# jedisct1/zig-lz4

Measured on AMD Instinct MI355X. Metric: GiB/s uncompressed, block compress+decompress, higher is better.
Workload: dtype u8

## Files before the change

### zig-lz4_amd/csrc/zlz4_compress_dict.hip

```cpp
#include "zlz4_device.hpp"

namespace zlz4 {

namespace {

__device__ __forceinline__ uint32_t dc_hash4(uint32_t seq) { return (seq * kHashMul) >> 20; }

__device__ __forceinline__ uint32_t dc_skip_sum(uint32_t x) {
    const uint32_t q = x >> 6, r = x & 63u;
    return 32u * q * (q - 1u) + q * r;
}

__device__ __forceinline__ int64_t dc_last_literals(uint8_t *dst, uint32_t dst_len, uint32_t op, const uint8_t *lit_src,
                                                    uint32_t lit, uint32_t lane) {
    if (lit == 0) return (int64_t)op;
    const uint32_t nle = ext_len_bytes(lit);
    if ((uint64_t)op + 1u + nle + lit > dst_len) return kErrOutputTooSmall;
    if (lane == 0) dst[op] = (uint8_t)((lit >= 15u ? 15u : lit) << 4);
    if (lit >= 15u) write_ext_len(dst + op + 1u, lit, lane);
    copy_bytes(dst + op + 1u + nle, lit_src, lit, lane);
    return (int64_t)(op + 1u + nle + lit);
}

struct VBuf {
// ... 275 lines not shown
                    if (x >= 64u) {
                        if (nseq == 0u) continue_generic = true;
                        break;
                    }
                    uint64_t pm = 0;
                    if (xp >> 7) {
                        const uint64_t grp_x = (uint64_t)rdlane((uint32_t)grp, x) | ((uint64_t)rdlane((uint32_t)(grp >> 32), x) << 32);
                        pm = grp_x & wrmask & ~covered_now() & ((1ull << x) - 1ull);
                    }
                    const uint32_t j = x;
                    const uint32_t m_pos = A + j;
                    uint32_t m_cand, mlen;
                    if (pm) {
                        const uint32_t pr = 63u - (uint32_t)__builtin_clzll(pm);
                        if (rdlane(fwd.x, pr) != rdlane(fwd.x, x)) { f = x + 1u; continue; }
                        m_cand = A + pr;
                        const uint64_t xa = ((uint64_t)(rdlane(fwd.z, j) ^ rdlane(fwd.z, pr)) << 32) | (rdlane(fwd.y, j) ^ rdlane(fwd.y, pr));
                        const uint32_t xb = rdlane(fwd.w, j) ^ rdlane(fwd.w, pr);
                        if (xa) mlen = (uint32_t)__builtin_ctzll(xa) >> 3;
                        else if (xb) mlen = 8u + ((uint32_t)__builtin_ctz(xb) >> 3);
                        else mlen = dc_extend_match(V, m_pos, m_cand, 12u, match_limit, lane);
                    } else {
                        const uint32_t q = rdlane(Q, x);
                        if (!(q & 1u)) { f = x + 1u; continue; }
                        mlen = q >> 1;
                        if (mlen < 44u && !tight) {
                            mm_run |= 1ull << j;
                            nseq++;
                            a = j + kMinMatch + mlen;
                            if (a >= 64u) break;
                            f = a + 1u;
                            continue;
                        }
                        m_cand = rdlane(old, x);
                        if (mlen >= 44u) mlen = dc_extend_match(V, m_pos, m_cand, 44u, match_limit, lane);
                    }
                    const uint32_t lit = j - a;
                    const uint32_t offset = m_pos - m_cand;
                    const uint32_t e = j + kMinMatch + mlen;
                    if (!tight && mlen < 270u) {
                        v_end = wrlane(e, j, v_end);
                        mlo_e = wrlane(mlen, j, mlo_e);
                        off_e = wrlane(offset, j, off_e);
                        mm_run |= 1ull << j;
                        nseq++;
                        a = e;
                        if (e >= 64u) break;
                        f = e + 1u;
                        continue;
                    }
                    if (mm_run) flush_run();
                    const uint32_t nle = ext_len_bytes(lit), nme = ext_len_bytes(mlen);
                    const uint64_t seq_end = (uint64_t)op + 1u + nle + lit + 2u + nme;
                    if (seq_end > dst_len) { failed = true; break; }
                    if (lane == 0)
                        dst[op] = (uint8_t)(((lit >= 15u ? 15u : lit) << 4) | (mlen >= 15u ? 15u : mlen));
                    if (lit >= 15u) write_ext_len(dst + op + 1u, lit, lane);
                    uint8_t *o = dst + op + 1u + nle;
                    if (lane >= a && lane < j) o[lane - a] = (uint8_t)fwd.x;
                    o += lit;
                    if (lane < 2u) o[lane] = (uint8_t)(offset >> (8u * lane));
                    if (mlen >= 15u) write_ext_len(o + 2u, mlen, lane);
                    op = (uint32_t)seq_end;
                    {
                        const uint64_t upto_e = e >= 64u ? ~0ull : (1ull << e) - 1ull;
                        covered_x |= upto_e & ~((2ull << j) - 1ull);
                    }
                    nseq++;
                    a = e;
                    if (e >= 64u) break;
                    f = e + 1u;
                }
                const bool next_win = !continue_generic && !failed && a != 0u && (uint64_t)A + a + 192u < L;
                if (next_win) {
                    pf_anchor = A + a;
                    fwd_pf = ld128(V.srcv + pf_anchor + lane);
                }
                if (mm_run && !failed) flush_run();
                anchor = A + a;
                const uint32_t f_end = continue_generic ? 64u : (a >= 64u ? 64u : a + 1u);
                const uint64_t ins = wrmask & ~covered_now() & (f_end >= 64u ? ~0ull : (1ull << f_end) - 1ull);
                if (failed) break;
                if (wr && !(ins & lane_bit)) table[h] = (T)old;
                __builtin_amdgcn_fence(__ATOMIC_RELEASE, "wavefront");
                if ((ins & lane_bit) && (grp & ins & ~lanes_below & ~lane_bit) == 0) table[h] = (T)mine;
                __builtin_amdgcn_fence(__ATOMIC_RELEASE, "wavefront");
                moved = anchor != A;
                to_generic = continue_generic;
                if (next_win) {
                    has_ins = true;
                    F0 = anchor + 1u;
                    if (++guard > src_size) { failed = true; break; }
                    continue;
                }
                break;
              }
                if (failed) break;
                if (!to_generic && moved) {
                    if (anchor < L) { has_ins = true; F0 = anchor + 1u; }
                    else { has_ins = false; F0 = L; }
                    continue;
                }
                if (to_generic) ub = 63;
            }

            bool found = false;
            uint32_t m_pos = 0, m_cand = 0, m_local = 0;
            bool m_local_done = false;
            for (;;) {
                const int32_t u = ub + (int32_t)lane;
                uint32_t pos, step_next;
                if (u <= 0) {
                    pos = (u < 0) ? F0 - 1u : F0;
                    step_next = accel;
                } else if (u == 1) {
                    pos = F0 + accel;
                    step_next = accel >> 6;
                } else {
                    const uint32_t x = cbase + (uint32_t)u - 1u;
                    pos = F0 + accel + dc_skip_sum(x) - s_cbase;
                    step_next = x >> 6;
                }
                const bool is_probe = u >= 0;
                const bool bail = is_probe && ((uint64_t)pos + step_next > L);
                const uint64_t bail_mask = ballot(bail);
                const uint32_t nb = bail_mask ? first_lane(bail_mask) : 64u;
                const bool active = lane < nb;

                const bool have16 = active && (pos + 16u <= V.end);
                u32x4 fwd = {0, 0, 0, 0};
                if (have16) fwd = ld128(V.srcv + pos);
                else if (active) fwd.x = ld32(V.srcv + pos);
                const uint32_t h = dc_hash4(fwd.x);
                const uint32_t mine = (uint32_t)(T)pos;

                uint32_t old = 0, rb = 0;
                if (active) {
                    old = table[h];
                    table[h] = (T)mine;
                }
                __builtin_amdgcn_fence(__ATOMIC_RELEASE, "wavefront");
                if (active) rb = table[h];
                uint64_t losers = ballot(active && rb != mine);
                uint64_t grp = lane_bit;
                int32_t pred = -1;
                while (losers) {
                    const uint32_t l = first_lane(losers);
                    const uint32_t hh = rdlane(h, l);
                    const uint64_t same = ballot(active && h == hh);
                    if (active && h == hh) {
                        grp = same;
                        const uint64_t below = same & lanes_below;
                        pred = below ? 63 - (int32_t)__clzll((long long)below) : -1;
                    }
                    losers &= ~same;
                }
                const uint32_t pred_pos = shfl(pos, (uint32_t)(pred < 0 ? 0 : pred));
                const uint32_t cand = pred >= 0 ? pred_pos : old;

                bool valid = is_probe && active && cand > 0 && cand < pos && (cand + kMaxDist >= pos);
                u32x4 cnd = {0, 0, 0, 0};
                bool cnd16 = false;
                if (valid) {
                    cnd16 = have16 && V.whole(cand, 16u);
                    if (cnd16) cnd = ld128(V.at(cand)); else cnd.x = V.rd32(cand);
                    valid = cnd.x == fwd.x;
                }
                const uint64_t valid_mask = ballot(valid);

                if (valid_mask) {
                    const uint32_t wl = first_lane(valid_mask);
                    if (active && lane > wl) table[h] = (T)old;
                    __builtin_amdgcn_fence(__ATOMIC_RELEASE, "wavefront");
                    const uint64_t upto = (2ull << wl) - 1ull;
                    if (active && lane <= wl && ((grp & upto & ~lanes_below & ~lane_bit) == 0)) table[h] = (T)mine;
                    __builtin_amdgcn_fence(__ATOMIC_RELEASE, "wavefront");
                    uint32_t loc = 0;
                    bool loc_done = false;
                    if (lane == wl && cnd16) {
                        const uint32_t lim = match_limit - (pos + kMinMatch);
                        u32x4 a = fwd, b = cnd;
                        a.x = 0; b.x = 0;
                        loc = first_diff16(a, b) - 4u;
                        if (loc >= lim) { loc = lim; loc_done = true; }
                        else if (loc < 12u) loc_done = true;
                    }
                    m_pos = rdlane(pos, wl);
                    m_cand = rdlane(cand, wl);
                    m_local = rdlane(loc, wl);
                    m_local_done = rdlane((uint32_t)loc_done, wl) != 0;
                    found = true;
                    break;
                }
                if (bail_mask) break;
                if (active && ((grp & ~lanes_below & ~lane_bit) == 0) && grp != lane_bit) table[h] = (T)mine;
                __builtin_amdgcn_fence(__ATOMIC_RELEASE, "wavefront");
                ub += 64;
            }
            if (!found) break;

            const uint32_t mlen = m_local_done ? m_local : dc_extend_match(V, m_pos, m_cand, m_local, match_limit, lane);

            const uint32_t lit = m_pos - anchor;
            const uint32_t nle = ext_len_bytes(lit), nme = ext_len_bytes(mlen);
            const uint64_t seq_end = (uint64_t)op + 1u + nle + lit + 2u + nme;
            if (seq_end > dst_len) { failed = true; break; }
            if (lane == 0)
                dst[op] = (uint8_t)(((lit >= 15u ? 15u : lit) << 4) | (mlen >= 15u ? 15u : mlen));
            if (lit >= 15u) write_ext_len(dst + op + 1u, lit, lane);
            uint8_t *o = dst + op + 1u + nle;
            copy_bytes(o, V.srcv + anchor, lit, lane);
            o += lit;
            const uint32_t offset = m_pos - m_cand;
            if (lane < 2u) o[lane] = (uint8_t)(offset >> (8u * lane));
            if (mlen >= 15u) write_ext_len(o + 2u, mlen, lane);
            op = (uint32_t)seq_end;

            const uint32_t end = m_pos + kMinMatch + mlen;
            anchor = end;
            if (end < L) { has_ins = true; F0 = end + 1u; }
            else { has_ins = false; F0 = L; }
        }
        res = failed ? kErrOutputTooSmall
                     : dc_last_literals(dst, dst_len, op, V.srcv + anchor, V.end - anchor, lane);
    }
    if (lane == 0) d_result[blk] = res;
}

}

extern "C" int zlz4_launch_compress_fast_using_dict(hipStream_t stream, const uint8_t *d_in, const uint64_t *d_in_off,
                                                    const uint32_t *d_in_len, uint8_t *d_out, const uint64_t *d_out_off,
                                                    const uint32_t *d_out_cap, const uint8_t *d_dict,
                                                    const uint64_t *d_dict_off, const uint32_t *d_dict_len,
                                                    const uint32_t *d_table, const uint32_t *d_table_idx, int64_t *d_result,
                                                    uint32_t nblocks, uint32_t max_in_len, uint32_t max_dict_len,
                                                    uint32_t acceleration) {
    if (nblocks == 0) return 0;
    const uint32_t dmax = max_dict_len < 65536u ? max_dict_len : 65536u;
#define ZLZ4_LAUNCH_DICT(T)                                                                                              \
    hipLaunchKernelGGL((zlz4::k_compress_fast_dict<T>), dim3(nblocks), dim3(64), 4096 * sizeof(T), stream, d_in, d_in_off, \
                       d_in_len, d_out, d_out_off, d_out_cap, d_dict, d_dict_off, d_dict_len, d_table, d_table_idx,        \
                       d_result, nblocks, max_in_len, dmax, acceleration)
    if ((uint64_t)dmax + max_in_len <= 65536u + 11u) ZLZ4_LAUNCH_DICT(uint16_t);
    else ZLZ4_LAUNCH_DICT(uint32_t);
#undef ZLZ4_LAUNCH_DICT
    return hipGetLastError() == hipSuccess ? 0 : -7;
}
```

### zig-lz4_amd/csrc/zlz4_compress_fast.hip

```cpp
#include <cstdlib>

#include "zlz4_device.hpp"

#ifdef ZLZ4_STAMPS
__device__ unsigned long long g_zlz4_stamps[24];
#define STAMP_DECL unsigned long long st_acc[24] = {0,0,0,0,0,0,0,0,0,0,0,0,0,0,0,0,0,0,0,0,0,0,0,0}; unsigned long long st_last = __builtin_amdgcn_s_memtime();
#define STAMP(i) do { unsigned long long st_now; __builtin_amdgcn_sched_barrier(0); \
                      asm volatile("s_memtime %0\n\ts_waitcnt lgkmcnt(0)" : "=s"(st_now) :: "memory"); \
                      __builtin_amdgcn_sched_barrier(0); st_acc[i] += st_now - st_last; st_last = st_now; } while (0)
#define STAMP_COUNT(i) do { st_acc[i] += 1; } while (0)
#define STAMP_FLUSH do { if (lane == 0) for (int st_k = 0; st_k < 24; st_k++) atomicAdd(&g_zlz4_stamps[st_k], st_acc[st_k]); } while (0)
#else
#define STAMP_DECL
#define STAMP(i)
#define STAMP_COUNT(i)
#define STAMP_FLUSH
#endif

namespace zlz4 {

__device__ __forceinline__ uint32_t hash4(uint32_t seq) { return (seq * kHashMul) >> 20; }

__device__ __forceinline__ uint32_t skip_sum(uint32_t x) {
    const uint32_t q = x >> 6, r = x & 63u;
// ... 84 lines not shown
                }
                for (int q = 0; q < 4; q++) table[4u * k + q] = (T)e[q];
            }
            __builtin_amdgcn_fence(__ATOMIC_RELEASE, "wavefront");
        } else {
        {
            u32x4 z = {0, 0, 0, 0};
            u32x4 *t4 = reinterpret_cast<u32x4 *>(lds_raw) + wave_in_wg * (4096u * sizeof(T) / 16u);
            const uint32_t n16 = 4096u * sizeof(T) / 16u;
            for (uint32_t k = lane; k < n16; k += 64u) t4[k] = z;
        }
        }
        const uint32_t accel = acceleration < 1u ? 1u : (acceleration > 65537u ? 65537u : acceleration);
        const uint32_t cbase = accel > 64u ? accel : 64u;
        const uint32_t s_cbase = skip_sum(cbase);
        const uint32_t L = src_size - kMfLimit;
        const uint32_t match_limit = src_size - kLastLiterals;
        const uint64_t lane_bit = 1ull << lane;
        const uint64_t lanes_below = lane_bit - 1ull;

        uint32_t anchor = 0, op = 0;
        uint32_t F0 = 1;
        bool has_ins = false;
        bool failed = false;
        STAMP_DECL
        STAMP(0);

        uint32_t guard = 0;

        constexpr bool kRing = sizeof(T) == 2;
        uint32_t rpos = 0x80000000u + 4u * lane;
        uint32_t r0 = 0, r1 = 0, r2 = 0;
        uint32_t ring_lim = 0;
        if constexpr (kRing) asm volatile("v_mov_b32 %0, %1" : "=v"(ring_lim) : "s"(src_size - 4u));
        auto ring_q = [&](uint32_t q) -> uint32_t { return q < ring_lim ? q : ring_lim; };
        auto ring_win = [&](uint32_t A) -> uint32_t {
            uint32_t rel = rfl(A - rpos);
            if (rel >= 256u) {
                const bool reload = rel >= 512u;
                const uint32_t nb = reload ? (A & ~127u) + 4u * lane : rpos + 256u;
                asm volatile("s_waitcnt vmcnt(0)\n\t"
                             "s_cmpk_lt_u32 %[rel], 0x200\n\t"
                             "s_cbranch_scc1 1f\n\t"
                             "global_load_dword %[r0], %[q0], %[src]\n\t"
                             "global_load_dword %[r1], %[q1], %[src]\n\t"
                             "s_waitcnt vmcnt(0)\n\t"
                             "s_branch 2f\n"
                             "1:\n\t"
                             "v_mov_b32 %[r0], %[r1]\n\t"
                             "v_mov_b32 %[r1], %[r2]\n"
                             "2:\n\t"
                             "global_load_dword %[r2], %[q2], %[src]"
                             : [r0] "+v"(r0), [r1] "+v"(r1), [r2] "+v"(r2)
                             : [rel] "s"(rel), [q0] "v"(ring_q(nb)), [q1] "v"(ring_q(nb + 256u)), [q2] "v"(ring_q(nb + 512u)),
                               [src] "s"(src)
                             : "scc", "memory");
                rpos = nb;
                rel = reload ? A & 127u : rel - 256u;
            }
            const uint32_t s0 = rel >> 2;
            return shfl(lane >= s0 ? r0 : r1, (s0 + lane) & 63u);
        };
        auto win_bytes = [&](uint32_t W, uint32_t A, uint32_t k0, uint32_t *out, uint32_t n) {
            const uint32_t o = (A & 3u) + lane, jw = (o >> 2) + k0;
            uint32_t lo = shfl(W, jw);
            for (uint32_t k = 0; k < n; k++) {
                const uint32_t hi = shfl(W, jw + k + 1u);
                out[k] = __builtin_amdgcn_alignbyte(hi, lo, o & 3u);
                lo = hi;
            }
        };
        auto ring_fwd = [&](uint32_t W, uint32_t A) -> u32x4 {
            uint32_t d[4];
            win_bytes(W, A, 0u, d, 4u);
            return u32x4{d[0], d[1], d[2], d[3]};
        };
        u32x4 fwd_pf = {0, 0, 0, 0};
        uint32_t w_pf = 0;
        uint32_t pf_anchor = 0xFFFFFFFFu;
        while (F0 < L) {
            if (++guard > src_size) { failed = true; break; }
            int32_t ub = -1;

            if (accel == 1u && F0 == anchor + 1u && (has_ins || anchor == 0u) && (uint64_t)anchor + 192u < L) {
              bool moved = false;
              bool to_generic = false;
              for (;;) {
                const uint32_t A = anchor;
                const uint32_t pos = A + lane;
                const bool wr = has_ins || lane > 0;
                if (kRing && pf_anchor != A) {
                    w_pf = ring_win(A);
                    fwd_pf = ring_fwd(w_pf, A);
                }
                const uint32_t W = w_pf;
                const u32x4 fwd = (kRing || pf_anchor == A) ? fwd_pf : ld128(src + pos);
                const uint32_t prod = fwd.x * kHashMul;
                const uint32_t h = prod >> 20;
                const uint32_t tg = (prod >> 12) & 0xFFu;
                const uint32_t mine = kTag == 2 ? (pos | (tg << 24)) : (uint32_t)(T)pos;
                STAMP(1);
                STAMP_COUNT(16);
                uint32_t old_e = 0, rb = 0, told = tg;
                if (wr) {
                    old_e = table[h];
                    if (kTag == 1) told = tags[h];
                }
                if (kTag == 2) told = old_e >> 24;
                const uint32_t old = old_e & kPosMask;
                const bool old_ok = wr && old > 0 && (!kSeed || old < pos) && (old + kMaxDist >= pos) && (kTag == 0 || told == tg);
                u32x4 cold = {0, 0, 0, 0};
                if (old_ok) cold = ld128(src + old);
                constexpr bool kGuess2 = sizeof(T) == 4;
                const uint32_t old12 = kGuess2 ? shfl(old, (lane + 12u) & 63u) : 0u;
                const bool pred2 = kGuess2 && old_ok && lane < 52u && old12 == old + 12u;
                u32x4 f2 = {0, 0, 0, 0}, c2 = f2, f3 = f2, c3 = f2;
                if (pred2) {
                    if (!kRing) { f2 = ld128(src + pos + 16u); f3 = ld128(src + pos + 32u); }
                    c2 = ld128(src + old + 16u); c3 = ld128(src + old + 32u);
                }
                STAMP(3);
                if (wr) table[h] = (T)mine;
                __builtin_amdgcn_fence(__ATOMIC_RELEASE, "wavefront");
                if (wr) rb = table[h];
                uint64_t losers = ballot(wr && rb != mine);
                uint64_t grp = lane_bit;
                while (losers) {
                    const uint32_t l = first_lane(losers);
                    const uint32_t hh = rdlane(h, l);
                    const uint64_t same = ballot(wr && h == hh);
                    if (wr && h == hh) grp = same;
                    losers &= ~same;
                }
                STAMP(2);

                const bool vo = old_ok && cold.x == fwd.x;
                uint32_t mlo;
                {
                    const uint32_t x1 = fwd.y ^ cold.y, x2 = fwd.z ^ cold.z, x3 = fwd.w ^ cold.w;
                    const uint32_t xs = x1 ? x1 : (x2 ? x2 : x3);
                    const uint32_t xbase = x1 ? 0u : (x2 ? 4u : 8u);
                    mlo = xs ? xbase + ((uint32_t)__builtin_ctz(xs) >> 3) : 12u;
                }
                const bool need2 = vo && mlo == 12u;
                if (need2 && !pred2) {
                    if (!kRing) { f2 = ld128(src + pos + 16u); f3 = ld128(src + pos + 32u); }
                    c2 = ld128(src + old + 16u); c3 = ld128(src + old + 32u);
                }
                if (kRing && ballot(need2)) {
                    uint32_t d[8];
                    win_bytes(W, A, 4u, d, 8u);
                    f2 = u32x4{d[0], d[1], d[2], d[3]};
                    f3 = u32x4{d[4], d[5], d[6], d[7]};
                }
                if (need2) {
                    const uint32_t d2 = first_diff16_sel(f2, c2);
                    mlo += d2 == 16u ? 16u + first_diff16_sel(f3, c3) : d2;
                }
                const bool single = (grp & lanes_below) == 0;
                const bool oldfast = vo && mlo < 44u;
                const uint64_t wrmask = ballot(wr);
                const uint64_t cfast = ballot(oldfast);
                const uint64_t slow = ballot(wr && ((!single && !oldfast) || (vo && mlo >= 44u)));
                const uint64_t nsing = ballot(wr && !single);
                uint32_t J, S;
                {
                    const uint64_t mj = cfast >> lane, ms = slow >> lane;
                    J = mj ? lane + (uint32_t)__builtin_ctzll(mj) : 64u;
                    S = ms ? lane + (uint32_t)__builtin_ctzll(ms) : 64u;
                }
                uint32_t v_end = lane + kMinMatch + mlo;
                uint32_t mlo_e = mlo, off_e = pos - old;
                uint32_t XP, Q;
                {
                    const uint32_t xm = J < S ? J : S;
                    XP = xm | ((uint32_t)((nsing >> (xm & 63u)) & 1ull) << 7);
                    Q = (vo ? 1u : 0u) | (mlo << 1);
                }
                uint32_t PK;
                {
                    const uint32_t jc = J & 63u;
                    const uint32_t ve_j = shfl(v_end, jc);
                    const bool fastok = J < 64u && S > J && !((nsing >> jc) & 1ull);
                    PK = fastok ? (J | (ve_j << 6)) : 0xFFFFFFFFu;
                }

                STAMP(6);
                uint32_t f = 1;
                uint32_t a = 0;
                uint32_t nseq = 0;
                uint64_t covered_x = 0;
                uint64_t mm_win = 0;
                bool continue_generic = false;
                const bool tight = dst_len - op < 512u;
                uint32_t a0 = a, op0 = op;
                uint64_t mm_run = 0;
                auto covered_now = [&]() -> uint64_t {
                    const uint64_t mb = (mm_win | mm_run) & lanes_below;
                    const uint32_t pj = mb ? 63u - (uint32_t)__builtin_clzll(mb) : 0u;
                    const uint32_t pe = shfl(v_end, pj);
                    return covered_x | ballot(mb != 0 && lane < pe);
                };
                auto flush_run = [&]() {
                    STAMP(9); STAMP_COUNT(21);
                    const uint64_t mb = mm_run & lanes_below;
                    const bool has_prev = mb != 0;
                    const uint32_t pj = has_prev ? 63u - (uint32_t)__builtin_clzll(mb) : 0u;
                    const uint32_t pend_all = shfl(v_end, pj);
                    const uint32_t pend = has_prev ? pend_all : a0;
                    const bool cov = has_prev && lane < pend_all;
                    const bool is_m = (mm_run & lane_bit) != 0;
                    const uint32_t jlast = 63u - (uint32_t)__builtin_clzll(mm_run);
                    const bool is_lit = lane >= a0 && lane < jlast && !cov && !is_m;
                    const uint64_t litmask = ballot(is_lit);
                    const uint64_t extm = ballot(is_m && mlo_e >= 15u);
                    const uint64_t at_or_above = mm_run & ~lanes_below;
                    const uint32_t my_m = at_or_above ? (uint32_t)__builtin_ctzll(at_or_above) : lane;
                    const uint32_t own_l = (my_m - pend >= 15u) ? 1u : 0u;
                    const uint64_t lextm = ballot(is_m && own_l != 0u);
                    const uint32_t k = (uint32_t)__popcll(mb);
                    const uint32_t lb = (uint32_t)__popcll(litmask & lanes_below);
                    const uint32_t o1 = op0 + 3u * k + lb + 1u + (uint32_t)__popcll(extm & lanes_below) +
                                        (uint32_t)__popcll(lextm & lanes_below) + own_l;
                    if (is_lit) dst[o1] = (uint8_t)fwd.x;
                    if (is_m) {
                        const uint32_t lit_k = lane - pend;
                        uint8_t *tk = dst + (o1 - 1u - lit_k - own_l);
                        tk[0] = (uint8_t)(((lit_k < 15u ? lit_k : 15u) << 4) | (mlo_e < 15u ? mlo_e : 15u));
                        if (own_l) tk[1] = (uint8_t)(lit_k - 15u);
                        const uint16_t off16 = (uint16_t)off_e;
                        __builtin_memcpy(dst + o1, &off16, 2);
                        if (mlo_e >= 15u) dst[o1 + 2u] = (uint8_t)(mlo_e - 15u);
                    }
                    const uint32_t nm = (uint32_t)__popcll(mm_run);
                    op = op0 + 3u * nm + (uint32_t)__popcll(litmask) + (uint32_t)__popcll(extm) + (uint32_t)__popcll(lextm);
                    mm_win |= mm_run;
                    mm_run = 0;
                    STAMP(10);
                };
                for (;;) {
                    if (mm_run == 0) { a0 = a; op0 = op; }
                    if (!tight) {
                        uint32_t t_pk, t_j;
#define ZLZ4_FAST_RUN_TRIP                                   \
                            "s_cmp_gt_u32 %[f], 63\n\t"      \
                            "s_cbranch_scc1 3f\n\t"          \
                            "v_readlane_b32 %[pk], %[PK], %[f]\n\t" \
                            "s_cmp_eq_u32 %[pk], -1\n\t"     \
                            "s_cbranch_scc1 3f\n\t"          \
                            "s_lshr_b32 %[a], %[pk], 6\n\t"  \
                            "s_add_u32 %[f], %[a], 1\n\t"    \
                            "s_and_b32 %[j], %[pk], 63\n\t"  \
                            "s_bitset1_b64 %[mm], %[j]\n\t"  \
                            "s_add_u32 %[nseq], %[nseq], 1\n\t"
                        asm volatile(
                            "s_nop 3\n"
                            "1:\n\t"
                            ZLZ4_FAST_RUN_TRIP
                            ZLZ4_FAST_RUN_TRIP
                            "s_branch 1b\n"
                            "3:\n"
                            : [f] "+s"(f), [a] "+s"(a), [nseq] "+s"(nseq), [mm] "+s"(mm_run), [pk] "=&s"(t_pk), [j] "=&s"(t_j)
                            : [PK] "v"(PK)
                            : "scc");
#undef ZLZ4_FAST_RUN_TRIP
                    }
                    STAMP(8);
                    if (f >= 64u) {
                        if (nseq == 0u) continue_generic = true;
                        break;
                    }

                    const uint32_t xp = rdlane(XP, f);
                    const uint32_t x = xp & 127u;
                    if (x >= 64u) {
                        if (nseq == 0u) continue_generic = true;
                        break;
                    }
                    uint64_t pm = 0;
                    if (xp >> 7) {
                        const uint64_t grp_x = (uint64_t)rdlane((uint32_t)grp, x) | ((uint64_t)rdlane((uint32_t)(grp >> 32), x) << 32);
                        pm = grp_x & wrmask & ~covered_now() & ((1ull << x) - 1ull);
                    }
                    const uint32_t j = x;
                    const uint32_t m_pos = A + j;
                    uint32_t m_cand, mlen;
                    if (pm) {
                        const uint32_t pr = 63u - (uint32_t)__builtin_clzll(pm);
                        if (rdlane(fwd.x, pr) != rdlane(fwd.x, x)) { STAMP_COUNT(19); STAMP(9); f = x + 1u; continue; }
                        STAMP_COUNT(18);
                        m_cand = A + pr;
                        const uint64_t xa = ((uint64_t)(rdlane(fwd.z, j) ^ rdlane(fwd.z, pr)) << 32) | (rdlane(fwd.y, j) ^ rdlane(fwd.y, pr));
                        const uint32_t xb = rdlane(fwd.w, j) ^ rdlane(fwd.w, pr);
                        if (xa) mlen = (uint32_t)__builtin_ctzll(xa) >> 3;
                        else if (xb) mlen = 8u + ((uint32_t)__builtin_ctz(xb) >> 3);
                        else mlen = extend_match(src, m_pos, m_cand, 12u, match_limit, src_size, lane);
                    } else {
                        const uint32_t q = rdlane(Q, x);
                        if (!(q & 1u)) { STAMP_COUNT(19); STAMP(9); f = x + 1u; continue; }
                        STAMP_COUNT(18);
                        mlen = q >> 1;
                        if (mlen < 44u && !tight) {
                            mm_run |= 1ull << j;
                            nseq++;
                            a = j + kMinMatch + mlen;
                            STAMP(9);
                            if (a >= 64u) break;
                            f = a + 1u;
                            continue;
                        }
                        m_cand = rdlane(old, x);
                        if (mlen >= 44u) mlen = extend_match(src, m_pos, m_cand, 44u, match_limit, src_size, lane);
                    }
                    const uint32_t lit = j - a;
                    const uint32_t offset = m_pos - m_cand;
                    const uint32_t e = j + kMinMatch + mlen;
                    if (!tight && mlen < 270u) {
                        v_end = wrlane(e, j, v_end);
                        mlo_e = wrlane(mlen, j, mlo_e);
                        off_e = wrlane(offset, j, off_e);
                        mm_run |= 1ull << j;
                        nseq++;
                        a = e;
                        STAMP(9);
                        if (e >= 64u) break;
                        f = e + 1u;
                        continue;
                    }
                    if (mm_run) flush_run();
                    const uint32_t nle = ext_len_bytes(lit), nme = ext_len_bytes(mlen);
                    const uint64_t seq_end = (uint64_t)op + 1u + nle + lit + 2u + nme;
                    if (seq_end > dst_len) { failed = true; break; }
                    if (lane == 0)
                        dst[op] = (uint8_t)(((lit >= 15u ? 15u : lit) << 4) | (mlen >= 15u ? 15u : mlen));
                    if (lit >= 15u) write_ext_len(dst + op + 1u, lit, lane);
                    uint8_t *o = dst + op + 1u + nle;
                    if (lane >= a && lane < j) o[lane - a] = (uint8_t)fwd.x;
                    o += lit;
                    if (lane < 2u) o[lane] = (uint8_t)(offset >> (8u * lane));
                    if (mlen >= 15u) write_ext_len(o + 2u, mlen, lane);
                    op = (uint32_t)seq_end;
                    {
                        const uint64_t upto_e = e >= 64u ? ~0ull : (1ull << e) - 1ull;
                        covered_x |= upto_e & ~((2ull << j) - 1ull);
                    }
                    nseq++;
                    a = e;
                    if (e >= 64u) break;
                    f = e + 1u;
                }
                const bool next_win = !continue_generic && !failed && a != 0u && (uint64_t)A + a + 192u < L;
                if (next_win) {
                    pf_anchor = A + a;
                    if constexpr (kRing) {
                        w_pf = ring_win(pf_anchor);
                        fwd_pf = ring_fwd(w_pf, pf_anchor);
                    } else {
                        fwd_pf = ld128(src + pf_anchor + lane);
                    }
                }
                if (mm_run && !failed) flush_run();
                anchor = A + a;
                STAMP(4);
                const uint32_t f_end = continue_generic ? 64u : (a >= 64u ? 64u : a + 1u);
                const uint64_t ins = wrmask & ~covered_now() & (f_end >= 64u ? ~0ull : (1ull << f_end) - 1ull);
                if (failed) break;
                if (wr && !(ins & lane_bit)) table[h] = (T)old_e;
                __builtin_amdgcn_fence(__ATOMIC_RELEASE, "wavefront");
                if ((ins & lane_bit) && (grp & ins & ~lanes_below & ~lane_bit) == 0) {
                    table[h] = (T)mine;
                    if (kTag == 1) tags[h] = (uint8_t)tg;
                }
                __builtin_amdgcn_fence(__ATOMIC_RELEASE, "wavefront");
                STAMP(5);
                moved = anchor != A;
                to_generic = continue_generic;
                if (next_win) {
                    has_ins = true;
                    F0 = anchor + 1u;
                    if (++guard > src_size) { failed = true; break; }
                    continue;
                }
                break;
              }
                if (failed) break;
                if (!to_generic && moved) {
                    if (anchor < L) { has_ins = true; F0 = anchor + 1u; }
                    else { has_ins = false; F0 = L; }
                    continue;
                }
                if (to_generic) ub = 63;
            }

            bool found = false, bailed = false;
            uint32_t m_pos = 0, m_cand = 0, m_local = 0;
            bool m_local_done = false;
            for (;;) {
                const int32_t u = ub + (int32_t)lane;
                uint32_t pos, step_next;
                if (u <= 0) {
                    pos = (u < 0) ? F0 - 1u : F0;
                    step_next = accel;
                } else if (u == 1) {
                    pos = F0 + accel;
                    step_next = accel >> 6;
                } else {
                    const uint32_t x = cbase + (uint32_t)u - 1u;
                    pos = F0 + accel + skip_sum(x) - s_cbase;
                    step_next = x >> 6;
                }
                const bool is_probe = u >= 0;
                const bool bail = is_probe && ((uint64_t)pos + step_next > L);
                const uint64_t bail_mask = ballot(bail);
                const uint32_t nb = bail_mask ? first_lane(bail_mask) : 64u;
                const bool active = (lane < nb) && (is_probe || has_ins);

                const bool have16 = active && (pos + 16u <= src_size);
                u32x4 fwd = {0, 0, 0, 0};
                if (have16) fwd = ld128(src + pos);
                else if (active) fwd.x = ld32(src + pos);
                const uint32_t prod = fwd.x * kHashMul;
                const uint32_t h = prod >> 20;
                const uint32_t tg = (prod >> 12) & 0xFFu;
                const uint32_t mine = kTag == 2 ? (pos | (tg << 24)) : (uint32_t)(T)pos;

                uint32_t old_e = 0, rb = 0, told = tg;
                if (active) {
                    old_e = table[h];
                    if (kTag == 1) told = tags[h];
                    table[h] = (T)mine;
                }
                if (kTag == 2) told = old_e >> 24;
                const uint32_t old = old_e & kPosMask;
                __builtin_amdgcn_fence(__ATOMIC_RELEASE, "wavefront");
                if (active) rb = table[h];
                uint64_t losers = ballot(active && rb != mine);
                uint64_t grp = lane_bit;
                int32_t pred = -1;
                while (losers) {
                    const uint32_t l = first_lane(losers);
                    const uint32_t hh = rdlane(h, l);
                    const uint64_t same = ballot(active && h == hh);
                    if (active && h == hh) {
                        grp = same;
                        const uint64_t below = same & lanes_below;
                        pred = below ? 63 - (int32_t)__clzll((long long)below) : -1;
                    }
                    losers &= ~same;
                }
                const uint32_t pred_pos = shfl(pos, (uint32_t)(pred < 0 ? 0 : pred));
                const uint32_t cand = pred >= 0 ? pred_pos : old;

                bool valid = is_probe && active && cand > 0 && cand < pos && (cand + kMaxDist >= pos) &&
                             (kTag == 0 || pred >= 0 || told == tg);
                u32x4 cnd = {0, 0, 0, 0};
                if (valid) {
                    if (have16) cnd = ld128(src + cand); else cnd.x = ld32(src + cand);
                    valid = cnd.x == fwd.x;
                }
                const uint64_t valid_mask = ballot(valid);

                if (valid_mask) {
                    const uint32_t wl = first_lane(valid_mask);
                    if (active && lane > wl) table[h] = (T)old_e;
                    __builtin_amdgcn_fence(__ATOMIC_RELEASE, "wavefront");
                    const uint64_t upto = (2ull << wl) - 1ull;
                    if (active && lane <= wl && ((grp & upto & ~lanes_below & ~lane_bit) == 0)) {
                        table[h] = (T)mine;
                        if (kTag == 1) tags[h] = (uint8_t)tg;
                    }
                    uint32_t loc = 0;
                    bool loc_done = false;
                    if (lane == wl) {
                        const uint32_t lim = match_limit - (pos + kMinMatch);
                        if (have16) {
                            u32x4 a = fwd, b = cnd;
                            a.x = 0; b.x = 0;
                            loc = first_diff16(a, b) - 4u;
                            if (loc >= lim) { loc = lim; loc_done = true; }
                            else if (loc < 12u) loc_done = true;
                        }
                    }
                    m_pos = rdlane(pos, wl);
                    m_cand = rdlane(cand, wl);
                    m_local = rdlane(loc, wl);
                    m_local_done = rdlane((uint32_t)loc_done, wl) != 0;
                    found = true;
                    break;
                }
                if (bail_mask) {
                    if constexpr (kSeed) {
                        if (active && ((grp & ~lanes_below & ~lane_bit) == 0) && grp != lane_bit) table[h] = (T)mine;
                        __builtin_amdgcn_fence(__ATOMIC_RELEASE, "wavefront");
                    }
                    bailed = true; break;
                }
                if (active && ((grp & ~lanes_below & ~lane_bit) == 0)) {
                    if (grp != lane_bit) table[h] = (T)mine;
                    if (kTag == 1) tags[h] = (uint8_t)tg;
                }
                __builtin_amdgcn_fence(__ATOMIC_RELEASE, "wavefront");
                ub += 64;
            }
            if (bailed || !found) break;
            STAMP_COUNT(20);

            const uint32_t mlen = m_local_done ? m_local
                                               : extend_match(src, m_pos, m_cand, m_local, match_limit, src_size, lane);

            const uint32_t lit = m_pos - anchor;
            const uint32_t nle = ext_len_bytes(lit), nme = ext_len_bytes(mlen);
            const uint64_t seq_end = (uint64_t)op + 1u + nle + lit + 2u + nme;
            if (seq_end > dst_len) { failed = true; break; }
            if (lane == 0)
                dst[op] = (uint8_t)(((lit >= 15u ? 15u : lit) << 4) | (mlen >= 15u ? 15u : mlen));
            if (lit >= 15u) write_ext_len(dst + op + 1u, lit, lane);
            uint8_t *o = dst + op + 1u + nle;
            copy_bytes(o, src + anchor, lit, lane);
            o += lit;
            const uint32_t offset = m_pos - m_cand;
            if (lane < 2u) o[lane] = (uint8_t)(offset >> (8u * lane));
            if (mlen >= 15u) write_ext_len(o + 2u, mlen, lane);
            op = (uint32_t)seq_end;

            const uint32_t end = m_pos + kMinMatch + mlen;
            anchor = end;
            if (end < L) { has_ins = true; F0 = end + 1u; }
            else { has_ins = false; F0 = L; }
        }
        if constexpr (kRing) asm volatile("s_waitcnt vmcnt(0)" : "+v"(r2));
        if constexpr (kSeed) {
            if (!failed && has_ins && F0 >= L && lane == 0) {
                const uint32_t prod = ld32(src + anchor) * kHashMul;
                table[prod >> 20] = (T)(kTag == 2 ? (anchor | ((prod >> 12 & 0xFFu) << 24)) : anchor);
            }
        }
        res = failed ? kErrOutputTooSmall
                     : emit_last_literals(dst, dst_len, op, src + anchor, src_size - anchor, lane);
        STAMP(7);
        STAMP_FLUSH;
    }
    if constexpr (kSeed) {
        if (d_table_out) {
            const uint32_t tix = d_table_idx ? rfl(d_table_idx[blk]) : blk;
            const uint32_t *seed = d_table_in + (uint64_t)tix * 4096u;
            uint32_t *out = d_table_out + (uint64_t)blk * 4096u;
            const bool merged = src_size >= kMfLimit + 1u && src_size <= max_in_len && src_size <= kMaxInput && res >= 0;
            if (merged) {
// ... 110 lines not shown
```

### zig-lz4_amd/csrc/zlz4_device.hpp

```cpp
#pragma once
#include <hip/hip_runtime.h>
#include <stdint.h>
#include <stdlib.h>

#ifdef ZLZ4_TUNING
static inline const char *zlz4_tune_env(const char *name) { return getenv(name); }
#else
static inline const char *zlz4_tune_env(const char *) { return nullptr; }
#endif

namespace zlz4 {

typedef uint32_t u32x4 __attribute__((ext_vector_type(4)));
typedef uint32_t u32x2 __attribute__((ext_vector_type(2)));

constexpr uint32_t kMinMatch = 4;
constexpr uint32_t kLastLiterals = 5;
constexpr uint32_t kMfLimit = 12;
constexpr uint32_t kMaxInput = 0x7E000000u;
constexpr uint32_t kMaxDist = 65535u;
constexpr uint32_t kHashMul = 2654435761u;

constexpr int64_t kErrOutputTooSmall = -1;
constexpr int64_t kErrInputTooLarge = -2;
constexpr int64_t kErrCorrupted = -3;
constexpr int64_t kErrInvalidState = -5;

constexpr uint32_t kBoundSkip = 0xFFFFFFFFu, kBoundInvalid = 0xFFFFFFFEu, kBoundMax = 0xFFFF0000u;

__device__ __forceinline__ uint32_t rfl(uint32_t v) { return __builtin_amdgcn_readfirstlane(v); }
__device__ __forceinline__ uint32_t rdlane(uint32_t v, uint32_t l) { return __builtin_amdgcn_readlane(v, l); }
__device__ __forceinline__ uint64_t ballot(bool p) { return __ballot(p); }
__device__ __forceinline__ uint32_t first_lane(uint64_t m) { return (uint32_t)__ffsll((long long)m) - 1u; }
__device__ __forceinline__ uint32_t shfl(uint32_t v, uint32_t src_lane) {
    return (uint32_t)__builtin_amdgcn_ds_bpermute((int)(src_lane << 2), (int)v);
}

__device__ __forceinline__ uint32_t wrlane(uint32_t val, uint32_t l, uint32_t old) {
    return (__lane_id() == l) ? val : old;
}

__device__ __forceinline__ uint32_t ld32(const uint8_t *p) { uint32_t v; __builtin_memcpy(&v, p, 4); return v; }
__device__ __forceinline__ u32x4 ld128(const uint8_t *p) { u32x4 v; __builtin_memcpy(&v, p, 16); return v; }
__device__ __forceinline__ void st128(uint8_t *p, u32x4 v) { __builtin_memcpy(p, &v, 16); }

__device__ __forceinline__ uint32_t first_diff16(u32x4 a, u32x4 b) {
    const uint32_t x0 = a.x ^ b.x, x1 = a.y ^ b.y, x2 = a.z ^ b.z, x3 = a.w ^ b.w;
    if (x0) return (uint32_t)__builtin_ctz(x0) >> 3;
    if (x1) return 4u + ((uint32_t)__builtin_ctz(x1) >> 3);
    if (x2) return 8u + ((uint32_t)__builtin_ctz(x2) >> 3);
    if (x3) return 12u + ((uint32_t)__builtin_ctz(x3) >> 3);
    return 16u;
}

__device__ __forceinline__ uint32_t first_diff16_sel(u32x4 a, u32x4 b) {
    const uint32_t x0 = a.x ^ b.x, x1 = a.y ^ b.y, x2 = a.z ^ b.z, x3 = a.w ^ b.w;
    const uint32_t lo = x0 ? x0 : x1, hi = x2 ? x2 : x3;
    const uint32_t blo = x0 ? 0u : 4u, bhi = x2 ? 8u : 12u;
    const bool in_lo = (x0 | x1) != 0;
    const uint32_t x = in_lo ? lo : hi;
    const uint32_t base = in_lo ? blo : bhi;
    return x ? base + ((uint32_t)__builtin_ctz(x) >> 3) : 16u;
}

__device__ __forceinline__ void copy_bytes(uint8_t *dst, const uint8_t *src, uint32_t n, uint32_t lane) {
    uint32_t k = lane * 16u;
    for (; k + 16u <= n; k += 1024u) st128(dst + k, ld128(src + k));
    const uint32_t t0 = n & ~15u;
    if (t0 + lane < n && lane < 16u) dst[t0 + lane] = src[t0 + lane];
}

__device__ __forceinline__ uint32_t ext_len_bytes(uint32_t v) { return v >= 15u ? 1u + (v - 15u) / 255u : 0u; }

__device__ __forceinline__ void write_ext_len(uint8_t *p, uint32_t v, uint32_t lane) {
    const uint32_t rem = v - 15u;
    const uint32_t n255 = rem / 255u;
    for (uint32_t k = lane; k < n255; k += 64u) p[k] = 255;
    if (lane == 0) p[n255] = (uint8_t)(rem - n255 * 255u);
}

}
```

Baseline: 81.25.

## Restrict fast window path to has_ins and compute lane predicates as SGPR masks

The accelerated window path now requires has_ins, so the per-lane wr predicate disappears. The table write and readback are moved before the candidate loads. Per-lane booleans are rebuilt from scalar ballot masks via inverse_ballot, match-length search uses v_ffbl/min3, and covered-lane computation is merged into flush_run. A lanes_in_order helper adds a wave barrier and acquire fence between ordered table stores. The aim is fewer VALU instructions and VGPRs in the hot loop, at the cost of dropping the anchor==0 entry into the fast path and some risk to ordering semantics.

```diff
diff --git a/zig-lz4_amd/csrc/zlz4_compress_dict.hip b/zig-lz4_amd/csrc/zlz4_compress_dict.hip
--- a/zig-lz4_amd/csrc/zlz4_compress_dict.hip
+++ b/zig-lz4_amd/csrc/zlz4_compress_dict.hip
@@ -381,7 +381,7 @@
                 const uint64_t ins = wrmask & ~covered_now() & (f_end >= 64u ? ~0ull : (1ull << f_end) - 1ull);
                 if (failed) break;
                 if (wr && !(ins & lane_bit)) table[h] = (T)old;
-                __builtin_amdgcn_fence(__ATOMIC_RELEASE, "wavefront");
+                lanes_in_order();
                 if ((ins & lane_bit) && (grp & ins & ~lanes_below & ~lane_bit) == 0) table[h] = (T)mine;
                 __builtin_amdgcn_fence(__ATOMIC_RELEASE, "wavefront");
                 moved = anchor != A;
@@ -470,7 +470,7 @@
                 if (valid_mask) {
                     const uint32_t wl = first_lane(valid_mask);
                     if (active && lane > wl) table[h] = (T)old;
-                    __builtin_amdgcn_fence(__ATOMIC_RELEASE, "wavefront");
+                    lanes_in_order();
                     const uint64_t upto = (2ull << wl) - 1ull;
                     if (active && lane <= wl && ((grp & upto & ~lanes_below & ~lane_bit) == 0)) table[h] = (T)mine;
                     __builtin_amdgcn_fence(__ATOMIC_RELEASE, "wavefront");
diff --git a/zig-lz4_amd/csrc/zlz4_compress_fast.hip b/zig-lz4_amd/csrc/zlz4_compress_fast.hip
--- a/zig-lz4_amd/csrc/zlz4_compress_fast.hip
+++ b/zig-lz4_amd/csrc/zlz4_compress_fast.hip
@@ -190,13 +190,12 @@
             if (++guard > src_size) { failed = true; break; }
             int32_t ub = -1;
 
-            if (accel == 1u && F0 == anchor + 1u && (has_ins || anchor == 0u) && (uint64_t)anchor + 192u < L) {
+            if (accel == 1u && has_ins && F0 == anchor + 1u && (uint64_t)anchor + 192u < L) {
               bool moved = false;
               bool to_generic = false;
               for (;;) {
                 const uint32_t A = anchor;
                 const uint32_t pos = A + lane;
-                const bool wr = has_ins || lane > 0;
                 if (kRing && pf_anchor != A) {
                     w_pf = ring_win(A);
                     fwd_pf = ring_fwd(w_pf, A);
@@ -209,14 +208,18 @@
                 const uint32_t mine = kTag == 2 ? (pos | (tg << 24)) : (uint32_t)(T)pos;
                 STAMP(1);
                 STAMP_COUNT(16);
-                uint32_t old_e = 0, rb = 0, told = tg;
-                if (wr) {
-                    old_e = table[h];
-                    if (kTag == 1) told = tags[h];
-                }
+                uint32_t told = tg;
+                const uint32_t old_e = table[h];
+                if (kTag == 1) told = tags[h];
+                table[h] = (T)mine;
+                __builtin_amdgcn_fence(__ATOMIC_RELEASE, "wavefront");
+                const uint32_t rb = table[h];
                 if (kTag == 2) told = old_e >> 24;
                 const uint32_t old = old_e & kPosMask;
-                const bool old_ok = wr && old > 0 && (!kSeed || old < pos) && (old + kMaxDist >= pos) && (kTag == 0 || told == tg);
+                uint64_t m_ok = ballot(old > 0) & ballot(old + kMaxDist >= pos);
+                if (kSeed) m_ok &= ballot(old < pos);
+                if (kTag != 0) m_ok &= ballot(told == tg);
+                const bool old_ok = lane_of(m_ok);
                 u32x4 cold = {0, 0, 0, 0};
                 if (old_ok) cold = ld128(src + old);
                 constexpr bool kGuess2 = sizeof(T) == 4;
@@ -228,34 +231,28 @@
                     c2 = ld128(src + old + 16u); c3 = ld128(src + old + 32u);
                 }
                 STAMP(3);
-                if (wr) table[h] = (T)mine;
-                __builtin_amdgcn_fence(__ATOMIC_RELEASE, "wavefront");
-                if (wr) rb = table[h];
-                uint64_t losers = ballot(wr && rb != mine);
+                uint64_t losers = ballot(rb != mine);
                 uint64_t grp = lane_bit;
                 while (losers) {
                     const uint32_t l = first_lane(losers);
                     const uint32_t hh = rdlane(h, l);
-                    const uint64_t same = ballot(wr && h == hh);
-                    if (wr && h == hh) grp = same;
+                    const uint64_t same = ballot(h == hh);
+                    if (h == hh) grp = same;
                     losers &= ~same;
                 }
                 STAMP(2);
 
-                const bool vo = old_ok && cold.x == fwd.x;
-                uint32_t mlo;
-                {
-                    const uint32_t x1 = fwd.y ^ cold.y, x2 = fwd.z ^ cold.z, x3 = fwd.w ^ cold.w;
-                    const uint32_t xs = x1 ? x1 : (x2 ? x2 : x3);
-                    const uint32_t xbase = x1 ? 0u : (x2 ? 4u : 8u);
-                    mlo = xs ? xbase + ((uint32_t)__builtin_ctz(xs) >> 3) : 12u;
-                }
-                const bool need2 = vo && mlo == 12u;
+                const uint64_t m_vo = m_ok & ballot(cold.x == fwd.x);
+                const bool vo = lane_of(m_vo);
+                uint32_t mlo = min3u(ffbl(fwd.y ^ cold.y), ffbl(fwd.z ^ cold.z) | 32u, ffbl(fwd.w ^ cold.w) | 64u) >> 3;
+                mlo = mlo < 12u ? mlo : 12u;
+                const uint64_t m_need2 = m_vo & ballot(mlo == 12u);
+                const bool need2 = lane_of(m_need2);
                 if (need2 && !pred2) {
                     if (!kRing) { f2 = ld128(src + pos + 16u); f3 = ld128(src + pos + 32u); }
                     c2 = ld128(src + old + 16u); c3 = ld128(src + old + 32u);
                 }
-                if (kRing && ballot(need2)) {
+                if (kRing && m_need2) {
                     uint32_t d[8];
                     win_bytes(W, A, 4u, d, 8u);
                     f2 = u32x4{d[0], d[1], d[2], d[3]};
@@ -265,17 +262,15 @@
                     const uint32_t d2 = first_diff16_sel(f2, c2);
                     mlo += d2 == 16u ? 16u + first_diff16_sel(f3, c3) : d2;
                 }
-                const bool single = (grp & lanes_below) == 0;
-                const bool oldfast = vo && mlo < 44u;
-                const uint64_t wrmask = ballot(wr);
-                const uint64_t cfast = ballot(oldfast);
-                const uint64_t slow = ballot(wr && ((!single && !oldfast) || (vo && mlo >= 44u)));
-                const uint64_t nsing = ballot(wr && !single);
+                const uint64_t nsing = ballot((grp & lanes_below) != 0);
+                const uint64_t m_lt44 = ballot(mlo < 44u);
+                const uint64_t cfast = m_vo & m_lt44;
+                const uint64_t slow = (nsing & ~cfast) | (m_vo & ~m_lt44);
                 uint32_t J, S;
                 {
-                    const uint64_t mj = cfast >> lane, ms = slow >> lane;
-                    J = mj ? lane + (uint32_t)__builtin_ctzll(mj) : 64u;
-                    S = ms ? lane + (uint32_t)__builtin_ctzll(ms) : 64u;
+                    const uint64_t mj = cfast & ~lanes_below, ms = slow & ~lanes_below;
+                    J = min3u(ffbl((uint32_t)mj), ffbl((uint32_t)(mj >> 32)) | 32u, 64u);
+                    S = min3u(ffbl((uint32_t)ms), ffbl((uint32_t)(ms >> 32)) | 32u, 64u);
                 }
                 uint32_t v_end = lane + kMinMatch + mlo;
                 uint32_t mlo_e = mlo, off_e = pos - old;
@@ -289,7 +284,7 @@
                 {
                     const uint32_t jc = J & 63u;
                     const uint32_t ve_j = shfl(v_end, jc);
-                    const bool fastok = J < 64u && S > J && !((nsing >> jc) & 1ull);
+                    const bool fastok = J < S && XP < 128u;
                     PK = fastok ? (J | (ve_j << 6)) : 0xFFFFFFFFu;
                 }
 
@@ -303,30 +298,31 @@
                 const bool tight = dst_len - op < 512u;
                 uint32_t a0 = a, op0 = op;
                 uint64_t mm_run = 0;
+                auto prev_end = [&](uint64_t m) -> uint32_t {
+                    const uint64_t mb = m & lanes_below;
+                    const uint32_t pj = mb ? 63u - (uint32_t)__builtin_clzll(mb) : 0u;
+                    return shfl(v_end, pj);
+                };
                 auto covered_now = [&]() -> uint64_t {
-                    const uint64_t mb = (mm_win | mm_run) & lanes_below;
-                    const uint32_t pj = mb ? 63u - (uint32_t)__builtin_clzll(mb) : 0u;
-                    const uint32_t pe = shfl(v_end, pj);
-                    return covered_x | ballot(mb != 0 && lane < pe);
+                    const uint64_t m = mm_win | mm_run;
+                    return covered_x | (above_lowest(m) & ballot(lane < prev_end(m)));
                 };
-                auto flush_run = [&]() {
+                auto flush_run = [&]() -> uint64_t {
                     STAMP(9); STAMP_COUNT(21);
-                    const uint64_t mb = mm_run & lanes_below;
-                    const bool has_prev = mb != 0;
-                    const uint32_t pj = has_prev ? 63u - (uint32_t)__builtin_clzll(mb) : 0u;
-                    const uint32_t pend_all = shfl(v_end, pj);
-                    const uint32_t pend = has_prev ? pend_all : a0;
-                    const bool cov = has_prev && lane < pend_all;
-                    const bool is_m = (mm_run & lane_bit) != 0;
+                    const uint64_t m_all = mm_win | mm_run;
+                    const uint32_t pend_all = prev_end(m_all);
+                    const uint64_t inside = above_lowest(m_all) & ballot(lane < pend_all);
+                    const uint32_t pend = lane_of(above_lowest(mm_run)) ? pend_all : a0;
+                    const bool is_m = lane_of(mm_run);
                     const uint32_t jlast = 63u - (uint32_t)__builtin_clzll(mm_run);
-                    const bool is_lit = lane >= a0 && lane < jlast && !cov && !is_m;
-                    const uint64_t litmask = ballot(is_lit);
-                    const uint64_t extm = ballot(is_m && mlo_e >= 15u);
+                    const uint64_t litmask = ((1ull << jlast) - 1ull) & ~((1ull << a0) - 1ull) & ~inside & ~mm_run;
+                    const bool is_lit = lane_of(litmask);
+                    const uint64_t extm = mm_run & ballot(mlo_e >= 15u);
                     const uint64_t at_or_above = mm_run & ~lanes_below;
                     const uint32_t my_m = at_or_above ? (uint32_t)__builtin_ctzll(at_or_above) : lane;
                     const uint32_t own_l = (my_m - pend >= 15u) ? 1u : 0u;
-                    const uint64_t lextm = ballot(is_m && own_l != 0u);
-                    const uint32_t k = (uint32_t)__popcll(mb);
+                    const uint64_t lextm = mm_run & ballot(my_m - pend >= 15u);
+                    const uint32_t k = (uint32_t)__popcll(mm_run & lanes_below);
                     const uint32_t lb = (uint32_t)__popcll(litmask & lanes_below);
                     const uint32_t o1 = op0 + 3u * k + lb + 1u + (uint32_t)__popcll(extm & lanes_below) +
                                         (uint32_t)__popcll(lextm & lanes_below) + own_l;
@@ -342,9 +338,10 @@
                     }
                     const uint32_t nm = (uint32_t)__popcll(mm_run);
                     op = op0 + 3u * nm + (uint32_t)__popcll(litmask) + (uint32_t)__popcll(extm) + (uint32_t)__popcll(lextm);
-                    mm_win |= mm_run;
+                    mm_win = m_all;
                     mm_run = 0;
                     STAMP(10);
+                    return covered_x | inside;
                 };
                 for (;;) {
                     if (mm_run == 0) { a0 = a; op0 = op; }
@@ -388,7 +385,7 @@
                     uint64_t pm = 0;
                     if (xp >> 7) {
                         const uint64_t grp_x = (uint64_t)rdlane((uint32_t)grp, x) | ((uint64_t)rdlane((uint32_t)(grp >> 32), x) << 32);
-                        pm = grp_x & wrmask & ~covered_now() & ((1ull << x) - 1ull);
+                        pm = grp_x & ~covered_now() & ((1ull << x) - 1ull);
                     }
                     const uint32_t j = x;
                     const uint32_t m_pos = A + j;
@@ -467,15 +464,15 @@
                         fwd_pf = ld128(src + pf_anchor + lane);
                     }
                 }
-                if (mm_run && !failed) flush_run();
+                if (failed) break;
+                const uint64_t covered = mm_run ? flush_run() : covered_now();
                 anchor = A + a;
                 STAMP(4);
                 const uint32_t f_end = continue_generic ? 64u : (a >= 64u ? 64u : a + 1u);
-                const uint64_t ins = wrmask & ~covered_now() & (f_end >= 64u ? ~0ull : (1ull << f_end) - 1ull);
-                if (failed) break;
-                if (wr && !(ins & lane_bit)) table[h] = (T)old_e;
-                __builtin_amdgcn_fence(__ATOMIC_RELEASE, "wavefront");
-                if ((ins & lane_bit) && (grp & ins & ~lanes_below & ~lane_bit) == 0) {
+                const uint64_t ins = ~covered & (f_end >= 64u ? ~0ull : (1ull << f_end) - 1ull);
+                if (!lane_of(ins)) table[h] = (T)old_e;
+                lanes_in_order();
+                if (lane_of(ins) && (grp & ins & ~lanes_below & ~lane_bit) == 0) {
                     table[h] = (T)mine;
                     if (kTag == 1) tags[h] = (uint8_t)tg;
                 }
@@ -571,7 +568,7 @@
                 if (valid_mask) {
                     const uint32_t wl = first_lane(valid_mask);
                     if (active && lane > wl) table[h] = (T)old_e;
-                    __builtin_amdgcn_fence(__ATOMIC_RELEASE, "wavefront");
+                    lanes_in_order();
                     const uint64_t upto = (2ull << wl) - 1ull;
                     if (active && lane <= wl && ((grp & upto & ~lanes_below & ~lane_bit) == 0)) {
                         table[h] = (T)mine;
diff --git a/zig-lz4_amd/csrc/zlz4_device.hpp b/zig-lz4_amd/csrc/zlz4_device.hpp
--- a/zig-lz4_amd/csrc/zlz4_device.hpp
+++ b/zig-lz4_amd/csrc/zlz4_device.hpp
@@ -31,6 +31,15 @@
 __device__ __forceinline__ uint32_t rfl(uint32_t v) { return __builtin_amdgcn_readfirstlane(v); }
 __device__ __forceinline__ uint32_t rdlane(uint32_t v, uint32_t l) { return __builtin_amdgcn_readlane(v, l); }
 __device__ __forceinline__ uint64_t ballot(bool p) { return __ballot(p); }
+__device__ __forceinline__ void lanes_in_order() {
+    __builtin_amdgcn_fence(__ATOMIC_RELEASE, "wavefront");
+    __builtin_amdgcn_wave_barrier();
+    __builtin_amdgcn_fence(__ATOMIC_ACQUIRE, "wavefront");
+}
+__device__ __forceinline__ bool lane_of(uint64_t m) { return __builtin_amdgcn_inverse_ballot_w64(m); }
+__device__ __forceinline__ uint32_t ffbl(uint32_t x) { uint32_t r; asm("v_ffbl_b32 %0, %1" : "=v"(r) : "v"(x)); return r; }
+__device__ __forceinline__ uint32_t min3u(uint32_t a, uint32_t b, uint32_t c) { const uint32_t m = a < b ? a : b; return m < c ? m : c; }
+__device__ __forceinline__ uint64_t above_lowest(uint64_t m) { return ~(m ^ (m - 1ull)); }
 __device__ __forceinline__ uint32_t first_lane(uint64_t m) { return (uint32_t)__ffsll((long long)m) - 1u; }
 __device__ __forceinline__ uint32_t shfl(uint32_t v, uint32_t src_lane) {
     return (uint32_t)__builtin_amdgcn_ds_bpermute((int)(src_lane << 2), (int)v);
```

After: 87.91 (median of 6 runs). 1.08x the previous value.
